# OHDSI/bayes-bridge

Measured on AMD Instinct MI355X. Metric: Gibbs iters/sec (cg sampler), higher is better.
Workload: dtype f64

## Files before the change

bayes-bridge_amd/csrc/cg_sampler.hip:

```cpp
#include <sys/prctl.h>
#include <time.h>

#include "common.hpp"
#include "philox.hpp"
#include "tiled_layout.hpp"

namespace bbx {

int launch_cg_setup(bbx_design* h, int n_unshrunk, const double* phi,
                    const double* sd, const double* x0, double* s, double* d,
                    double* xs, CGState* st, double atol);
int launch_cg_direction(bbx_design* h, int k, CGState* st,
                        const double* rr_part, const double* r, double* pvec,
                        const double* s, double* sp, double* c_part,
                        const double* d = nullptr, double* pdp_part = nullptr,
                        unsigned long long* word = nullptr,
                        unsigned long long tag = 0);
int launch_cg_update(bbx_design* h, int k, CGState* st, const double* pq_part,
                     const double* pvec, const double* q, double* x, double* r,
                     double* rr_part);
int launch_cg_finish(bbx_design* h, const double* s, const double* x,
                     double* coef);

__global__ __launch_bounds__(256) void fill_normal_kernel(
// ... 15 lines not shown
    nz = nz || (x[i] != 0.);
  if (nz) atomicOr(flag, 1);
}

int launch_fill_normal(bbx_design* h, int64_t len, uint64_t seed,
                       uint64_t stream, double* d_out, bool prio,
                       hipStream_t on) {
  int64_t nb = (len + 255) / 256;
  if (nb > 4096) nb = 4096;
  if (nb < 1) nb = 1;
  BBX_LAUNCH(fill_normal_kernel, dim3((unsigned)nb), dim3(256), 0,
                     on ? on : h->stream, len, seed, stream, d_out,
                     prio ? 1 : 0);
  BBX_HIP(hipGetLastError());
  return BBX_OK;
}

struct CGUpdate {
  int k;
  CGState* st;
  double* x;
  double* r;
  bool* merged;
};
static int apply_operator(bbx_design* h, const double* d_omega,
                          const double* sp, const double* x, const double* s,
                          const double* d, double* q,
                          const CGUpdate* upd = nullptr) {
  TdotEpilogue ep;
  ep.mode = TD_OPER;
// ... 58 lines not shown
  double* sp = h->w_P[6].as<double>() + (h->intercept ? 1 : 0);
  CGState* st = h->cg_state.as<CGState>();
  const bool fold = tiled_fold_applies(h);
  double* sr = h->w_P[9].as<double>() + (h->intercept ? 1 : 0);
  double* tu = h->w_n[2].as<double>();

  if (d_eta1 == nullptr) {
    double* e1 = h->w_n[2].as<double>();
    double* e2 = h->w_P[8].as<double>();
    BBX_TRY(launch_fill_normal(h, h->n, seed, STREAM_ETA1, e1));
    BBX_TRY(launch_fill_normal(h, h->P, seed, STREAM_ETA2, e2));
    d_eta1 = e1;
    d_eta2 = e2;
  }

  BBX_TRY(launch_cg_setup(h, n_unshrunk, d_phi, d_sd, d_x0, s, d, x, st, atol));

  CGState* host_st = static_cast<CGState*>(h->host_pinned);
  if (x0_zero < 0) {
    int* d_flag = &st->pad;
    int* h_flag = reinterpret_cast<int*>(host_st);
    BBX_HIP(hipMemsetAsync(d_flag, 0, sizeof(int), h->stream));
    BBX_LAUNCH(any_nonzero_kernel, dim3(NPART), dim3(256), 0,
                       h->stream, h->P, d_x0, d_flag);
    BBX_HIP(hipGetLastError());
    BBX_HIP(hipMemcpyAsync(h_flag, d_flag, sizeof(int), hipMemcpyDeviceToHost,
                           h->stream));
    BBX_HIP(hipStreamSynchronize(h->stream));
    x0_zero = (*h_flag == 0) ? 1 : 0;
  }

// ... 1 lines not shown
    double* w = h->w_n[1].as<double>();
    TdotEpilogue ep;
    ep.mode = TD_RESID;
    ep.s = s;
    ep.d = d;
    ep.x = x0_zero ? nullptr : x;
    ep.z = d_z;
    ep.phi = d_phi;
    ep.eta2 = d_eta2;
    ep.dot_part = part_slot(h, PS_RR);
    if (fold) {
      ep.fold_sr = sr;
      ep.fold_cr_part = part_slot(h, PS_C);
    }
    if (!x0_zero && !h->sparse && dense_fused_applies(h)) {
      BBX_TRY(launch_prep_v(h, x, s, sp, part_slot(h, PS_C)));
      BBX_TRY(launch_sqrt_scale(h, d_omega, d_eta1, w, part_slot(h, PS_SUMW),
                                nullptr, true));
      const int st_f =
          launch_operator_dense_fused(h, sp, d_omega, ep, r, nullptr, w);
      if (st_f != 0)
        return st_f < 0 ? st_f
                        : fail(BBX_ERR_STATE,
                               "single-pass dense operator refused its design");
    } else {
      const double* t0 = nullptr;
      if (!x0_zero) {
        double* t = h->w_n[0].as<double>();
        BBX_TRY(launch_prep_v(h, x, s, sp, part_slot(h, PS_C)));
        BBX_TRY(launch_dot(h, sp, d_omega, t, nullptr));
        t0 = t;
      }
      BBX_TRY(launch_sqrt_scale(h, d_omega, d_eta1, w, part_slot(h, PS_SUMW),
                                t0, t0 == nullptr));
      BBX_TRY(launch_tdot(h, w, part_slot(h, PS_SUMW), ep, r));
    }
  }


  struct SkipScope {
    bbx_design* h;
    ~SkipScope() { h->skip_flag = nullptr; }
  } skip_scope{h};
  h->skip_flag = &st->done;
  double* pdp = part_slot(h, PS_PDP);
  bool merged = false;
  h->cg_serial += 1;
  const unsigned long long tag = (h->cg_serial & 0xFFFFFFull) << CG_WORD_TAG_SHIFT;
  unsigned long long* const word = h->cg_word_dev;
  volatile unsigned long long* const hword = h->cg_word_host;
  struct TagScope {
    bbx_design* h;
// ... 185 lines not shown
```

bayes-bridge_amd/csrc/chain.hip:

```cpp
#include <cmath>
#include <new>
#include <vector>

#include "chain.hpp"
#include "philox.hpp"
#include "samplers.hpp"
#include "pg_queue.hpp"

namespace bbx {

__device__ inline double wsum(double x) { return wave_allsum(x); }

__device__ inline double block_total_256(double x) {
  __shared__ double s_w[256 / WAVE];
  x = wsum(x);
  if ((threadIdx.x & (WAVE - 1)) == 0) s_w[threadIdx.x / WAVE] = x;
  __syncthreads();
  double r = 0.;
  if (threadIdx.x == 0)
    for (int k = 0; k < 256 / WAVE; ++k) r += s_w[k];
  __syncthreads();
  return r;
}

// ... 27 lines not shown
      prior_sd = shrunk_scale(g, lscale[j - nu], slab);
      guess *= prior_sd;
    }
    phi[j] = 1. / prior_sd;
    x0[j] = guess;
    double est = 1.;
    if (n_avg > 1) {
      const double k = (double)n_avg;
      const double m = mean[j];
      const double var = k / (k - 1.) * (square[j] - m * m);
      const double w = (k - 1.) / (k - 1. + 5.);
      est = sqrt(w * var + (1. - w) * 1.);
    }
    sd[j] = est;
    z[j] = zs * zbase[j];
  }
}

#define BBX_BRANCH_PRIO() do { if (prio) __builtin_amdgcn_s_setprio(3); } while (0)
static int lscale_prio() {
  static const int on = getenv("BBX_LSCALE_PRIO") ? atoi(getenv("BBX_LSCALE_PRIO")) : 1;
  return on;
}
static int branch_prio() {
  static const int on = !(getenv("BBX_BRANCH_PRIO") && atoi(getenv("BBX_BRANCH_PRIO")) == 0);
  return on;
}
__global__ __launch_bounds__(256) void chain_summary_kernel(
    int64_t P, int nu, double slab, long long n_avg,
    const ChainScalars* __restrict__ sc, const double* __restrict__ lscale,
// ... 129 lines not shown
    } else {
      const double xf = x / sd_unshrunk[j];
      c += xf * xf;
    }
  }
  const double ta = block_total_256(a);
  const double tb = block_total_256(b);
  const double tc = block_total_256(c);
  if (threadIdx.x == 0) {
    part_pow[blockIdx.x] = ta;
    part_slab[blockIdx.x] = tb;
    part_fixed[blockIdx.x] = tc;
  }
}

__global__ __launch_bounds__(256) void chain_gscale_kernel(
    int64_t n_shrunk, int nu, double alpha, double shape0, double rate0,
    double lower_bd, int update_mode, uint64_t seed, uint64_t stream,
    const double* __restrict__ part_pow, const double* __restrict__ part_slab,
    const double* __restrict__ part_fixed,
    const double* __restrict__ sd_unshrunk, ChainScalars* __restrict__ sc,
    int prio) {
  BBX_BRANCH_PRIO();
  const double pow_sum = sum_row_parts(part_pow, NPART);
  const double slab_sum = sum_row_parts(part_slab, NPART);
  const double fixed_sum = sum_row_parts(part_fixed, NPART);
  if (threadIdx.x != 0) return;
  double g = sc->gscale;
  if (n_shrunk > 0) {
    if (update_mode == BBX_GSCALE_OPTIMIZE) {
      const double ph = (double)n_shrunk / alpha / pow_sum;
      g = pow(ph, -(1. / alpha));
    } else if (update_mode == BBX_GSCALE_SAMPLE) {
      if (pow_sum == 0.) {
        g = 0.;
      } else {
        const double shape = shape0 + (double)n_shrunk / alpha;
        const double rate = rate0 + pow_sum;
        Philox rng(seed, stream, 0);
        const double ph = gamma_draw(rng, shape) / rate;
        g = 1. / pow(ph, 1. / alpha);
      }
    }
    if (update_mode != BBX_GSCALE_FIXED && g < lower_bd) {
      g = lower_bd;
      sc->n_gscale_clamped += 1;
    }
  } else {
    g = 1.;
  }
  sc->gscale = g;
  sc->abs_pow_sum = pow_sum;
  double lp = -.5 * slab_sum;
  double prior = 0.;
  if (n_shrunk > 0)
    prior += -(double)n_shrunk * log(g) - pow_sum / pow(g, alpha);
  prior += -.5 * fixed_sum;
  for (int j = 0; j < nu; ++j)
    if (sd_unshrunk[j] < INFINITY) prior -= log(sd_unshrunk[j]);
  prior += (shape0 - 1.) * log(g) - rate0 * g;
  sc->logprior = lp + prior;
}

constexpr int TS_BLOCK = 256;
constexpr int TS_MAX_COPIES = 16;
constexpr unsigned TS_MAX_TRIAL = 4095u;

template <class Store>
__device__ inline void tilted_stable_block(int64_t base, int64_t count,
                                           double a, uint64_t seed,
                                           uint64_t stream,
                                           const double* s_tilt,
                                           double cost_threshold, Store store) {
  __shared__ int s_pending[TS_BLOCK];
  __shared__ int s_next_dr[TS_BLOCK];
  __shared__ int s_next_dc[TS_BLOCK];
// ... 57 lines not shown
    if (active && ok && s_winner[item] == c) store(item, val);
    if (tid < m) {
      const int it = s_pending[tid];
      if (s_winner[it] == 0x7fffffff) {
        s_tried[it] += (unsigned)copies;
        if (tid < n_dr)
          s_next_dr[atomicAdd(&s_n_dr, 1)] = it;
        else
          s_next_dc[atomicAdd(&s_n_dc, 1)] = it;
      }
    }
    __syncthreads();
  }
}

__global__ __launch_bounds__(TS_BLOCK) void chain_lscale_kernel(
    int64_t n_shrunk, int nu, double alpha, uint64_t seed, uint64_t stream,
    ChainScalars* __restrict__ sc, const double* __restrict__ coef,
    double* __restrict__ lscale, int items, double cost_threshold, int prio) {
  __shared__ double s_tilt[TS_BLOCK];
  BBX_BRANCH_PRIO();
  const double g = sc->gscale;
  for (int64_t base = (int64_t)blockIdx.x * items; base < n_shrunk;
       base += (int64_t)gridDim.x * items) {
    const int64_t count =
        (n_shrunk - base < items) ? (n_shrunk - base) : items;
    if (alpha == 2.) {
      if (threadIdx.x < count) lscale[base + threadIdx.x] = .5;
      continue;
    }
    if (threadIdx.x < count) {
      const double r = coef[base + threadIdx.x + nu] / g;
      s_tilt[threadIdx.x] = r * r;
    }
    __syncthreads();
    tilted_stable_block(base, count, alpha / 2., seed, stream, s_tilt,
                        cost_threshold, [&](int item, double ts) {
// ... 68 lines not shown
static double ts_cost_threshold() { return TiltedStable::kCostThreshold; }

static inline uint64_t iter_stream(uint64_t stream, int64_t iter) {
  return stream | ((uint64_t)iter << 8);
}

static int grid_for(int64_t len, int cap) {
  int64_t nb = (len + 255) / 256;
  if (nb > cap) nb = cap;
  if (nb < 1) nb = 1;
  return (int)nb;
}

static int chain_linear_predictor(bbx_chain* c) {
  bbx_design* h = c->h;
  BBX_TRY(launch_prep_v(h, c->coef.as<double>(), nullptr, nullptr,
                        part_slot(h, PS_C), h->skip_flag));
  return launch_dot(h, c->coef.as<double>(), nullptr, c->psi.as<double>(),
                    nullptr);
}

static int chain_tail_hook(void* ctx) {
  return chain_linear_predictor(static_cast<bbx_chain*>(ctx));
}

static bool chain_tail_applies(const bbx_chain* c) {
  static const bool on = !(getenv("BBX_CHAIN_TAIL") && atoi(getenv("BBX_CHAIN_TAIL")) == 0);
  const bbx_design* h = c->h;
  if (!on || !h->sparse || h->format != BBX_FORMAT_TILED || h->hybrid) return false;
  int G = 0;
  return tiled_describe(h, 0, nullptr, nullptr, nullptr, &G, nullptr, nullptr) ==
             BBX_OK && G == 1;
// ... 17 lines not shown
                     c->n_unshrunk, c->model, c->slab,
                     (long long)c->n_averaged, sc, c->lscale.as<double>(),
                     c->sd_unshrunk.as<double>(), c->mean.as<double>(),
                     c->square.as<double>(), c->zbase.as<double>(),
                     c->phi.as<double>(), c->x0.as<double>(),
                     c->sd.as<double>(), c->z.as<double>(), c->pending_store,
                     c->samp_gscale.as<double>(), c->samp_logp.as<double>());
  c->pending_store = -1;
  if (c->model == BBX_MODEL_LINEAR)
    BBX_LAUNCH(chain_fill_obs_prec_kernel, dim3(grid_for(n, ROW_GRID)),
                       dim3(256), 0, s, n, sc, c->obs_prec.as<double>());
  BBX_HIP(hipGetLastError());
  return BBX_OK;
}

int chain_post_draw(bbx_chain* c, bool have_psi, int phases,
                    bbx_chain* branch_of) {
  bbx_design* h = c->h;
  hipStream_t s = h->stream;
  const int64_t P = h->P, n = h->n;
  const int nu = c->n_unshrunk;
  const int64_t n_shrunk = P - nu;
  ChainScalars* sc = c->scalars.as<ChainScalars>();

  static const int fork_env =
      getenv("BBX_CHAIN_FORK") ? atoi(getenv("BBX_CHAIN_FORK")) : -1;
  const bool fork = fork_env >= 0 ? fork_env == 1
                                  : (n >= 50000 && n_shrunk >= 2048);
  bbx_chain* owner = branch_of ? branch_of : c;
  if (fork && owner->stream2 == nullptr) {
    BBX_HIP(hipStreamCreateWithFlags(&owner->stream2, hipStreamNonBlocking));
  }
  if (fork && c->ev_join == nullptr)
    BBX_HIP(hipEventCreateWithFlags(&c->ev_join, hipEventDisableTiming));
  hipStream_t s_b = !fork ? s : owner->stream2;
  if (h->coef_in_flight) {
    if (fork && (phases & POST_BRANCH))
      BBX_HIP(hipStreamWaitEvent(s_b, h->ev_poll, 0));
    h->coef_in_flight = false;
  }

  if (!have_psi && (phases & POST_BRANCH)) BBX_TRY(chain_linear_predictor(c));

  if (phases & POST_BRANCH) {
  if (c->coef_sampler == BBX_SAMPLER_CG) {
    BBX_LAUNCH(chain_summary_kernel, dim3(NPART), dim3(256), 0, s_b, P,
                       nu, c->slab, (long long)c->n_averaged, sc,
                       c->lscale.as<double>(), c->coef.as<double>(),
                       c->mean.as<double>(), c->square.as<double>(),
                       fork ? branch_prio() : 0);
    c->n_averaged += 1;
  }
  double* pp = c->misc_part.as<double>();
  BBX_LAUNCH(chain_coef_sums_kernel, dim3(NPART), dim3(256), 0, s_b, P,
                     nu, c->bridge_exp, c->slab, c->coef.as<double>(),
                     c->sd_unshrunk.as<double>(), pp, pp + NPART,
                     pp + 2 * NPART, fork ? branch_prio() : 0);
  const double lower_bd = .001 / power_exp_ave_magnitude(c->bridge_exp);
  BBX_LAUNCH(chain_gscale_kernel, dim3(1), dim3(256), 0, s_b, n_shrunk,
                     nu, c->bridge_exp, c->shape0, c->rate0, lower_bd,
                     c->gscale_update, c->seed,
                     iter_stream(STREAM_GSCALE, c->iter), pp, pp + NPART,
                     pp + 2 * NPART, c->sd_unshrunk.as<double>(), sc,
                     fork ? branch_prio() : 0);
  if (n_shrunk > 0) {
    static const int items_env =
        getenv("BBX_TS_ITEMS") ? atoi(getenv("BBX_TS_ITEMS")) : 0;
    const int items = (items_env >= 8 && items_env <= TS_BLOCK) ? items_env
                      : (n_shrunk / TS_BLOCK < 1024) ? 128 : TS_BLOCK;
    int64_t nb = (n_shrunk + items - 1) / items;
    if (nb > 8192) nb = 8192;
    BBX_LAUNCH(chain_lscale_kernel, dim3((unsigned)nb), dim3(TS_BLOCK),
                       0, s_b, n_shrunk, nu, c->bridge_exp, c->seed,
                       iter_stream(STREAM_LSCALE, c->iter), sc,
                       c->coef.as<double>(), c->lscale.as<double>(), items,
                       ts_cost_threshold(), fork ? lscale_prio() : 0);
  }
  }

  hipError_t launch_err = hipSuccess;
  if (phases & POST_MAIN) {
  static const int eta_env =
      getenv("BBX_ETA_AHEAD") ? atoi(getenv("BBX_ETA_AHEAD")) : -1;
  const bool eta_ahead = eta_env >= 0 ? eta_env == 1 : n >= 250000;
  if (eta_ahead && fork && branch_of == nullptr && (phases & POST_JOIN)) {
    if (!c->eta1_next.ptr) {
      BBX_TRY(c->eta1_next.alloc(sizeof(double) * (size_t)n));
      BBX_TRY(c->eta2_next.alloc(sizeof(double) * (size_t)P));
    }
    const uint64_t next_seed = cg_draw_seed(c, (uint64_t)c->iter + 1);
    static const bool fill_prio = !(getenv("BBX_FILL_PRIO") &&
                                    atoi(getenv("BBX_FILL_PRIO")) == 0);
    BBX_TRY(launch_fill_normal(h, n, next_seed, STREAM_ETA1,
                               c->eta1_next.as<double>(), fill_prio));
    BBX_TRY(launch_fill_normal(h, P, next_seed, STREAM_ETA2,
                               c->eta2_next.as<double>(), fill_prio));
    c->eta_iter = c->iter + 1;
  }
  int rg = grid_for(n, ROW_GRID);
  double* rp = c->row_part.as<double>();
  if (c->model == BBX_MODEL_LOGIT) {
    static const int pg_env =
        getenv("BBX_PG_ELEMS") ? atoi(getenv("BBX_PG_ELEMS")) : -1;
    const int elems = pg_env >= 0 ? pg_env : polya_gamma_elems(n);
#define BBX_PG_LAUNCH(KERNEL, PER_BLOCK)                                       \
  do {                                                                         \
    rg = grid_for((n + (PER_BLOCK) - 1) / (PER_BLOCK) * 256, ROW_GRID);        \
    BBX_LAUNCH(KERNEL, dim3(rg), dim3(256), 0, s, n, c->seed,          \
                       iter_stream(STREAM_PG, c->iter),                        \
                       c->outcome.as<double>(), c->n_trial.as<double>(),       \
                       c->psi.as<double>(), c->obs_prec.as<double>(), rp);     \
  } while (0)
    if (elems == 0) BBX_PG_LAUNCH(chain_pg_lane_kernel, 256);
// ... 13 lines not shown

  launch_err = hipGetLastError();
  if (phases & POST_JOIN) {
    if (fork) {
      BBX_HIP(hipEventRecord(c->ev_join, s_b));
      BBX_HIP(hipStreamWaitEvent(s, c->ev_join, 0));
    }
    c->iter += 1;
  }
  BBX_HIP(launch_err);
  return BBX_OK;
}

static int chain_step(bbx_chain* c, int maxiter, double atol, int* n_cg_iter) {
  const uint64_t it = (uint64_t)c->iter;
  BBX_TRY(chain_pre_draw(c));
  int info = 0;
  const bool have_eta = c->eta_iter == (long long)it && c->eta1_next.ptr;
  if (c->coef_sampler == BBX_SAMPLER_CHOLESKY) {
    bbx_design* h = c->h;
    if (!have_eta) {
      if (!c->eta2_next.ptr)
        BBX_TRY(c->eta2_next.alloc(sizeof(double) * (size_t)h->P));
      BBX_TRY(launch_fill_normal(h, h->P, cg_draw_seed(c, it), STREAM_ETA2,
                                 c->eta2_next.as<double>()));
    }
    const bool linear = c->model == BBX_MODEL_LINEAR;
    const int st = chol_sample_device(
        h, linear ? nullptr : c->obs_prec.as<double>(), 1.,
        linear ? &c->scalars.as<ChainScalars>()->obs_prec : nullptr,
        c->phi.as<double>(), c->z.as<double>(), c->eta2_next.as<double>(),
        c->coef.as<double>());
    c->eta_iter = -1;
    if (st < 0) return st;
    c->coef_sample = nullptr;
    if (n_cg_iter) *n_cg_iter = 0;
    BBX_TRY(chain_post_draw(c, false, POST_ALL));
    return 0;
  }
  if (c->coef_sampler == BBX_SAMPLER_WOODBURY) {
    bbx_design* h = c->h;
    if (!have_eta) {
      if (!c->eta1_next.ptr)
        BBX_TRY(c->eta1_next.alloc(sizeof(double) * (size_t)h->n));
      if (!c->eta2_next.ptr)
        BBX_TRY(c->eta2_next.alloc(sizeof(double) * (size_t)h->P));
      BBX_TRY(launch_fill_normal(h, h->n, cg_draw_seed(c, it), STREAM_ETA1,
                                 c->eta1_next.as<double>()));
      BBX_TRY(launch_fill_normal(h, h->P, cg_draw_seed(c, it), STREAM_ETA2,
                                 c->eta2_next.as<double>()));
    }
    const bool linear = c->model == BBX_MODEL_LINEAR;
    const int st = woodbury_sample_device(
        h, linear ? nullptr : c->obs_prec.as<double>(), 1.,
        linear ? &c->scalars.as<ChainScalars>()->obs_prec : nullptr,
        c->phi.as<double>(),
        linear ? c->outcome.as<double>() : c->kappa.as<double>(),
        linear ? 0 : 1, c->eta1_next.as<double>(), c->eta2_next.as<double>(),
        c->coef.as<double>());
    c->eta_iter = -1;
    if (st < 0) return st;
    c->coef_sample = nullptr;
    if (n_cg_iter) *n_cg_iter = 0;
    BBX_TRY(chain_post_draw(c, false, POST_ALL));
    return 0;
  }
  struct TailScope {
    bbx_design* h;
    ~TailScope() {
      h->tail_hook = nullptr;
      h->tail_ctx = nullptr;
      h->coef_copy = nullptr;
    }
  } tail_scope{c->h};
  c->h->coef_copy = c->coef_sample;
  if (chain_tail_applies(c)) {
    c->h->tail_hook = chain_tail_hook;
    c->h->tail_ctx = c;
  }

  int st = cg_sample_device(
      c->h, c->obs_prec.as<double>(), c->phi.as<double>(), c->z.as<double>(),
      c->x0.as<double>(), c->sd.as<double>(), c->n_unshrunk,
      have_eta ? c->eta1_next.as<double>() : nullptr,
      have_eta ? c->eta2_next.as<double>() : nullptr,
      cg_draw_seed(c, it), maxiter, atol, c->coef.as<double>(), n_cg_iter,
      &info, c->mean_zero ? 1 : 0);
  c->eta_iter = -1;
  if (st < 0) return st;
  c->mean_zero = false;
  BBX_TRY(chain_post_draw(c, c->h->tail_ran, POST_ALL));
  c->h->tail_ran = false;
  return info;
}

int chain_begin_run(bbx_chain* c, int n_sample) {
  c->pending_store = -1;
  c->coef_sample = nullptr;
  BBX_TRY(c->samp_gscale.alloc(sizeof(double) * (size_t)(n_sample + 1)));
  BBX_TRY(c->samp_logp.alloc(sizeof(double) * (size_t)(n_sample + 1)));
  return BBX_OK;
}

int chain_save_sample(bbx_chain* c, int idx, double* d_coef, double* d_lscale,
                      double* d_obs_prec) {
  bbx_design* h = c->h;
  const int64_t P = h->P, n = h->n;
// ... 153 lines not shown
  *out = c;
  return BBX_OK;
}

int bbx_chain_destroy(bbx_chain* c) {
  if (!c) return BBX_OK;
  if (c->h && design_alive(c->h)) {
    (void)hipSetDevice(c->h->device);
    (void)hipStreamSynchronize(c->h->stream);
  }
  if (c->stream2) {
    (void)hipStreamSynchronize(c->stream2);
    (void)hipStreamDestroy(c->stream2);
  }
  if (c->ev_join) (void)hipEventDestroy(c->ev_join);
  if (c->pinned) (void)hipHostFree(c->pinned);
  delete c;
  return BBX_OK;
}

static int bbx_chain_set_state_impl(bbx_chain* c, const double* coef,
                        const double* obs_prec, const double* lscale,
                        const double* gscale) {
  BBX_TRY(chain_check(c));
  bbx_design* h = c->h;
  BBX_HIP(hipSetDevice(h->device));
  if (coef)
    BBX_HIP(hipMemcpy(c->coef.ptr, coef, sizeof(double) * (size_t)h->P,
                      hipMemcpyHostToDevice));
  ChainScalars sc;
// ... 457 lines not shown
```

bayes-bridge_amd/csrc/chain.hpp:

```cpp
#pragma once
#include <cmath>

#include "common.hpp"

namespace bbx {

constexpr int ROW_GRID = 2048;

struct alignas(128) ChainScalars {
  double gscale;
  double logprior;
  double abs_pow_sum;
  long long n_gscale_clamped;
  long long n_lscale_fixed;
  alignas(128) double obs_prec;
  double loglik;
  __host__ __device__ double logp() const { return loglik + logprior; }
};

}

struct bbx_chain {
  bbx_design* h = nullptr;
  int model = BBX_MODEL_LOGIT;
// ... 4 lines not shown
  int64_t n_averaged = 0;
  bool mean_zero = true;
  int gscale_update = BBX_GSCALE_SAMPLE;
  int coef_sampler = BBX_SAMPLER_CG;
  void (*progress)(int, void*) = nullptr;
  void* progress_ctx = nullptr;
  int progress_every = 0;
  bbx::DevMem outcome, n_trial, kappa;
  bbx::DevMem zbase;
  bbx::DevMem coef, phi, x0, sd, z, mean, square, sd_unshrunk;
  bbx::DevMem lscale;
  bbx::DevMem obs_prec, psi;
  bbx::DevMem scalars;
  bbx::DevMem row_part;
  bbx::DevMem misc_part;
  bbx::DevMem eta1_next, eta2_next;
  long long eta_iter = -1;
  bbx::DevMem samp_gscale, samp_logp;
  int pending_store = -1;
  double* coef_sample = nullptr;
  void* pinned = nullptr;
  hipStream_t stream2 = nullptr;
  hipEvent_t ev_join = nullptr;
};

namespace bbx {

inline uint64_t cg_draw_seed(const bbx_chain* c, uint64_t it) {
  return c->seed + 0x9E3779B97F4A7C15ull * (it + 1);
}

int chain_pre_draw(bbx_chain* c);
// ... 10 lines not shown
```

bayes-bridge_amd/csrc/common.hpp:

```cpp
#pragma once

#include <hip/hip_runtime.h>
#include <stdint.h>

#include <exception>
#include <new>
#include <string>
#include <vector>

#include "../../include/bbx.h"

#include <atomic>
namespace bbx {
extern std::atomic<unsigned long long> g_launch_count;
}
#define BBX_LAUNCH(...)                                                   \
  do {                                                                    \
    bbx::g_launch_count.fetch_add(1, std::memory_order_relaxed);          \
    hipLaunchKernelGGL(__VA_ARGS__);                                      \
  } while (0)
#define BBX_LAUNCH_EXT(...)                                               \
  do {                                                                    \
    bbx::g_launch_count.fetch_add(1, std::memory_order_relaxed);          \
    hipExtLaunchKernelGGL(__VA_ARGS__);                                   \
// ... 174 lines not shown
  bbx::DevMem cg_state;
  bbx::DevMem stage_n, stage_P;
  void* host_pinned = nullptr;

  int64_t n_dot = 0, n_tdot = 0;
  int last_cg_iter = 0;
  unsigned long long* cg_word_host = nullptr;
  unsigned long long* cg_word_dev = nullptr;
  unsigned long long cg_serial = 0;
  int cg_recent[8] = {0, 0, 0, 0, 0, 0, 0, 0};
  int cg_recent_n = 0;
  int64_t cg_period_ns = 0;
  bool coef_in_flight = false;
  int64_t cg_empty_launches = 0, cg_solves = 0, cg_naps = 0;
  double* coef_copy = nullptr;
  int (*tail_hook)(void*) = nullptr;
  void* tail_ctx = nullptr;
  bool tail_ran = false;
  hipEvent_t ev_poll = nullptr;
  bool in_operator = false;
  uint64_t operator_serial = 0;
  int cg_fold = -1;
  const int* skip_flag = nullptr;
  bbx::KernelTimer timer;
};

namespace bbx {

enum PartSlot {
  PS_C = 0,
// ... 187 lines not shown
                           const double* d_pps, const double* d_y, int y_is_wy,
                           const double* d_delta, const double* d_xi,
                           double* d_coef_out);
double* wb_stage(bbx_design* h, int k);
void woodbury_release(bbx_design* h);
int launch_dot_dense(bbx_design* h, const double* d_v, const double* d_rowscale,
                     double* d_t);
int launch_tdot_dense(bbx_design* h, const double* d_w, const double* d_sumw_part,
                      const TdotEpilogue& ep, double* d_out);
int cg_sample_device(bbx_design* h, const double* d_omega, const double* d_phi,
                     const double* d_z, const double* d_x0,
                     const double* d_sd, int n_unshrunk, const double* d_eta1,
                     const double* d_eta2, uint64_t seed, int maxiter,
                     double atol, double* d_coef, int* n_iter_out,
                     int* info_out, int x0_zero = -1);

}
```

bayes-bridge_amd/csrc/vecops.hip:

```cpp
#include "common.hpp"

namespace bbx {

std::atomic<unsigned long long> g_launch_count{0};


__device__ inline double wave_sum_v(double x) { return wave_allsum(x); }

__device__ inline void block_store_partial(double x, double* part) {
  __shared__ double s_w[VEC_BLOCK / WAVE];
  x = wave_sum_v(x);
  if ((threadIdx.x & (WAVE - 1)) == 0) s_w[threadIdx.x / WAVE] = x;
  __syncthreads();
  if (threadIdx.x == 0) {
    double r = 0.;
#pragma unroll
    for (int k = 0; k < VEC_BLOCK / WAVE; ++k) r += s_w[k];
    part[blockIdx.x] = r;
  }
  __syncthreads();
}

__device__ inline double sum_partials_v(const double* part) {
  __shared__ double s_tot;
// ... 99 lines not shown
                      const double* d_minus, bool negate) {
  BBX_LAUNCH(sqrt_scale_kernel, dim3(NPART), dim3(VEC_BLOCK), 0,
                     h->stream, h->n, d_omega, d_eta, d_w, d_part, d_minus,
                     negate ? 1 : 0);
  BBX_HIP(hipGetLastError());
  return BBX_OK;
}


__global__ __launch_bounds__(VEC_BLOCK) void cg_setup_kernel(
    int64_t P, int n_unshrunk, const double* __restrict__ phi,
    const double* __restrict__ sd, const double* __restrict__ x0,
    double* __restrict__ s, double* __restrict__ d, double* __restrict__ xs,
    CGState* __restrict__ st, double atol) {
  if (blockIdx.x == 0 && threadIdx.x == 0) {
    st->rho[0] = st->rho[1] = 0.;
    st->atol = atol;
    st->bnorm2 = 0.;
    st->n_iter = 0;
    st->done = 0;
    st->bad = 0;
    st->pad = 0;
    st->running = 1;
    st->pad2 = 0;
  }
  for (int64_t jj = (int64_t)blockIdx.x * VEC_BLOCK + threadIdx.x; jj < P;
       jj += (int64_t)gridDim.x * VEC_BLOCK) {
    const double ph = phi[jj];
    const double sj = (jj < n_unshrunk) ? 2. * sd[jj] : 1. / ph;
    const double sp = sj * ph;
    s[jj] = sj;
    d[jj] = sp * sp;
    xs[jj] = x0[jj] / sj;
  }
}

__global__ __launch_bounds__(VEC_BLOCK) void cg_direction_kernel(
    int64_t P, int intercept, int k, CGState* __restrict__ st,
    const double* __restrict__ rr_part, const double* __restrict__ r,
// ... 85 lines not shown
    const double rj = r0 - alpha * q0;
    r[j0] = rj;
    acc += rj * rj;
  }
  for (int64_t jj = j0 + stride; jj < P; jj += stride) {
    x[jj] += alpha * pvec[jj];
    const double rj = r[jj] - alpha * q[jj];
    r[jj] = rj;
    acc += rj * rj;
  }
  block_store_partial(acc, rr_part);
  if (blockIdx.x == 0 && threadIdx.x == 0) st->n_iter = k + 1;
}

__global__ __launch_bounds__(VEC_BLOCK) void cg_finish_kernel(
    int64_t P, const double* __restrict__ s, const double* __restrict__ x,
    double* __restrict__ coef, double* __restrict__ copy) {
  for (int64_t jj = (int64_t)blockIdx.x * VEC_BLOCK + threadIdx.x; jj < P;
       jj += (int64_t)gridDim.x * VEC_BLOCK) {
    const double v = s[jj] * x[jj];
    coef[jj] = v;
    if (copy) copy[jj] = v;
  }
}

int launch_cg_setup(bbx_design* h, int n_unshrunk, const double* phi,
                    const double* sd, const double* x0, double* s, double* d,
                    double* xs, CGState* st, double atol) {
  BBX_LAUNCH(cg_setup_kernel, dim3(NPART), dim3(VEC_BLOCK), 0,
                     h->stream, h->P, n_unshrunk, phi, sd, x0, s, d, xs, st,
                     atol);
  BBX_HIP(hipGetLastError());
  return BBX_OK;
}

int launch_cg_direction(bbx_design* h, int k, CGState* st,
                        const double* rr_part, const double* r, double* pvec,
                        const double* s, double* sp, double* c_part,
// ... 6 lines not shown
  return BBX_OK;
}

int launch_cg_update(bbx_design* h, int k, CGState* st, const double* pq_part,
                     const double* pvec, const double* q, double* x, double* r,
                     double* rr_part) {
  BBX_LAUNCH(cg_update_kernel, dim3(NPART), dim3(VEC_BLOCK), 0,
                     h->stream, h->P, k, st, pq_part, pvec, q, x, r, rr_part);
  BBX_HIP(hipGetLastError());
  return BBX_OK;
}

int launch_cg_finish(bbx_design* h, const double* s, const double* x,
                     double* coef) {
  BBX_LAUNCH(cg_finish_kernel, dim3(NPART), dim3(VEC_BLOCK), 0,
                     h->stream, h->P, s, x, coef, h->coef_copy);
  BBX_HIP(hipGetLastError());
  return BBX_OK;
}

}
```

Baseline: 331.1.

## Fuse chain setup with CG setup, fold gscale into lscale, prefetch next eta

Merges the per-iteration chain pre-draw and CG setup/prep kernels into one chain_setup_kernel. The finish kernel now also computes the offset partial dot, so the linear predictor can skip a prep pass. Coefficient summary and sums become one kernel, and the global-scale draw moves inside the local-scale kernel to drop a single-block launch. For large designs, the next iteration's normal draws are generated early on a side stream with double-buffered eta arrays. The aim is fewer launches and serial gaps per Gibbs step, at the cost of more coupling between stages and every block redundantly recomputing the gscale draw.

```diff
diff --git a/bayes-bridge_amd/csrc/cg_sampler.hip b/bayes-bridge_amd/csrc/cg_sampler.hip
--- a/bayes-bridge_amd/csrc/cg_sampler.hip
+++ b/bayes-bridge_amd/csrc/cg_sampler.hip
@@ -53,6 +53,17 @@
                      prio ? 1 : 0);
   BBX_HIP(hipGetLastError());
   return BBX_OK;
+}
+
+CGSetupTargets cg_setup_targets(const bbx_design* h) {
+  CGSetupTargets t;
+  t.s = h->w_P[0].as<double>();
+  t.d = h->w_P[1].as<double>();
+  t.xs = h->w_P[2].as<double>();
+  t.sp = h->w_P[6].as<double>() + (h->intercept ? 1 : 0);
+  t.c_part = part_slot(h, PS_C);
+  t.st = h->cg_state.as<CGState>();
+  return t;
 }
 
 struct CGUpdate {
@@ -141,7 +152,12 @@
     d_eta2 = e2;
   }
 
-  BBX_TRY(launch_cg_setup(h, n_unshrunk, d_phi, d_sd, d_x0, s, d, x, st, atol));
+  h->coef_c_ready = false;
+  const bool setup_done = h->setup_done;
+  if (setup_done && x0_zero < 0)
+    return fail(BBX_ERR_INVALID, "a caller's own set-up needs x0_zero given");
+  if (!setup_done)
+    BBX_TRY(launch_cg_setup(h, n_unshrunk, d_phi, d_sd, d_x0, s, d, x, st, atol));
 
   CGState* host_st = static_cast<CGState*>(h->host_pinned);
   if (x0_zero < 0) {
@@ -173,7 +189,7 @@
       ep.fold_cr_part = part_slot(h, PS_C);
     }
     if (!x0_zero && !h->sparse && dense_fused_applies(h)) {
-      BBX_TRY(launch_prep_v(h, x, s, sp, part_slot(h, PS_C)));
+      if (!setup_done) BBX_TRY(launch_prep_v(h, x, s, sp, part_slot(h, PS_C)));
       BBX_TRY(launch_sqrt_scale(h, d_omega, d_eta1, w, part_slot(h, PS_SUMW),
                                 nullptr, true));
       const int st_f =
@@ -186,7 +202,7 @@
       const double* t0 = nullptr;
       if (!x0_zero) {
         double* t = h->w_n[0].as<double>();
-        BBX_TRY(launch_prep_v(h, x, s, sp, part_slot(h, PS_C)));
+        if (!setup_done) BBX_TRY(launch_prep_v(h, x, s, sp, part_slot(h, PS_C)));
         BBX_TRY(launch_dot(h, sp, d_omega, t, nullptr));
         t0 = t;
       }
@@ -195,6 +211,7 @@
       BBX_TRY(launch_tdot(h, w, part_slot(h, PS_SUMW), ep, r));
     }
   }
+  if (h->resid_hook) BBX_TRY(h->resid_hook(h->resid_ctx));
 
 
   struct SkipScope {
diff --git a/bayes-bridge_amd/csrc/chain.hip b/bayes-bridge_amd/csrc/chain.hip
--- a/bayes-bridge_amd/csrc/chain.hip
+++ b/bayes-bridge_amd/csrc/chain.hip
@@ -65,6 +65,67 @@
     }
     sd[j] = est;
     z[j] = zs * zbase[j];
+  }
+}
+
+__global__ __launch_bounds__(256) void chain_setup_kernel(
+    int64_t P, int nu, int model, double slab, long long n_avg,
+    const ChainScalars* __restrict__ sc, const double* __restrict__ lscale,
+    const double* __restrict__ sd_unshrunk, const double* __restrict__ mean,
+    const double* __restrict__ square, const double* __restrict__ zbase,
+    double* __restrict__ phi, double* __restrict__ x0, double* __restrict__ sd,
+    double* __restrict__ z, int store_idx, double* __restrict__ samp_gs,
+    double* __restrict__ samp_lp, int intercept,
+    const double* __restrict__ offset, int warm, double* __restrict__ s,
+    double* __restrict__ d, double* __restrict__ xs, double* __restrict__ sp,
+    double* __restrict__ c_part, CGState* __restrict__ st, double atol) {
+  const double g = sc->gscale;
+  const double zs = (model == BBX_MODEL_LINEAR) ? sc->obs_prec : 1.;
+  if (blockIdx.x == 0 && threadIdx.x == 0) {
+    if (store_idx >= 0) {
+      samp_gs[store_idx] = g;
+      samp_lp[store_idx] = sc->logp();
+    }
+    cg_state_reset(st, atol);
+  }
+  double acc = 0.;
+  for (int64_t j = (int64_t)blockIdx.x * 256 + threadIdx.x; j < P;
+       j += (int64_t)gridDim.x * 256) {
+    double prior_sd, guess = mean[j];
+    if (j < nu) {
+      prior_sd = sd_unshrunk[j];
+    } else {
+      prior_sd = shrunk_scale(g, lscale[j - nu], slab);
+      guess *= prior_sd;
+    }
+    const double ph = 1. / prior_sd;
+    phi[j] = ph;
+    x0[j] = guess;
+    double est = 1.;
+    if (n_avg > 1) {
+      const double k = (double)n_avg;
+      const double m = mean[j];
+      const double var = k / (k - 1.) * (square[j] - m * m);
+      const double w = (k - 1.) / (k - 1. + 5.);
+      est = sqrt(w * var + (1. - w) * 1.);
+    }
+    sd[j] = est;
+    z[j] = zs * zbase[j];
+    const double sj = (j < nu) ? 2. * est : 1. / ph;
+    const double sph = sj * ph;
+    s[j] = sj;
+    d[j] = sph * sph;
+    const double xj = guess / sj;
+    xs[j] = xj;
+    if (warm) {
+      const double val = xj * sj;
+      sp[j] = val;
+      if (j >= intercept) acc += offset[j - intercept] * val;
+    }
+  }
+  if (warm) {
+    const double tot = block_total_256(acc);
+    if (threadIdx.x == 0) c_part[blockIdx.x] = tot;
   }
 }
 
@@ -224,19 +285,51 @@
   }
 }
 
-__global__ __launch_bounds__(256) void chain_gscale_kernel(
-    int64_t n_shrunk, int nu, double alpha, double shape0, double rate0,
-    double lower_bd, int update_mode, uint64_t seed, uint64_t stream,
-    const double* __restrict__ part_pow, const double* __restrict__ part_slab,
-    const double* __restrict__ part_fixed,
-    const double* __restrict__ sd_unshrunk, ChainScalars* __restrict__ sc,
-    int prio) {
+__global__ __launch_bounds__(256) void chain_summary_sums_kernel(
+    int64_t P, int nu, double alpha, double slab, long long n_avg,
+    int summarise, const ChainScalars* __restrict__ sc,
+    const double* __restrict__ lscale, const double* __restrict__ coef,
+    const double* __restrict__ sd_unshrunk, double* __restrict__ mean,
+    double* __restrict__ square, double* __restrict__ part_pow,
+    double* __restrict__ part_slab, double* __restrict__ part_fixed, int prio) {
   BBX_BRANCH_PRIO();
-  const double pow_sum = sum_row_parts(part_pow, NPART);
-  const double slab_sum = sum_row_parts(part_slab, NPART);
-  const double fixed_sum = sum_row_parts(part_fixed, NPART);
-  if (threadIdx.x != 0) return;
-  double g = sc->gscale;
+  const double g = sc->gscale;
+  const double w = 1. / (1. + (double)n_avg);
+  double a = 0., b = 0., c = 0.;
+  for (int64_t j = (int64_t)blockIdx.x * 256 + threadIdx.x; j < P;
+       j += (int64_t)gridDim.x * 256) {
+    const double x = coef[j];
+    if (summarise) {
+      double theta = x;
+      if (j >= nu) theta /= shrunk_scale(g, lscale[j - nu], slab);
+      mean[j] = w * theta + (1. - w) * mean[j];
+      square[j] = w * theta * theta + (1. - w) * square[j];
+    }
+    const double xs = x / slab;
+    b += xs * xs;
+    if (j >= nu) {
+      a += pow(fabs(x), alpha);
+    } else {
+      const double xf = x / sd_unshrunk[j];
+      c += xf * xf;
+    }
+  }
+  const double ta = block_total_256(a);
+  const double tb = block_total_256(b);
+  const double tc = block_total_256(c);
+  if (threadIdx.x == 0) {
+    part_pow[blockIdx.x] = ta;
+    part_slab[blockIdx.x] = tb;
+    part_fixed[blockIdx.x] = tc;
+  }
+}
+
+__device__ inline double gscale_draw(double g, int64_t n_shrunk, double alpha,
+                                     double shape0, double rate0,
+                                     double lower_bd, int update_mode,
+                                     uint64_t seed, uint64_t stream,
+                                     double pow_sum, bool* clamped) {
+  *clamped = false;
   if (n_shrunk > 0) {
     if (update_mode == BBX_GSCALE_OPTIMIZE) {
       const double ph = (double)n_shrunk / alpha / pow_sum;
@@ -254,11 +347,21 @@
     }
     if (update_mode != BBX_GSCALE_FIXED && g < lower_bd) {
       g = lower_bd;
-      sc->n_gscale_clamped += 1;
+      *clamped = true;
     }
   } else {
     g = 1.;
   }
+  return g;
+}
+
+__device__ inline void gscale_store(ChainScalars* __restrict__ sc, double g,
+                                    bool clamped, int64_t n_shrunk, int nu,
+                                    double alpha, double shape0, double rate0,
+                                    double pow_sum, double slab_sum,
+                                    double fixed_sum,
+                                    const double* __restrict__ sd_unshrunk) {
+  if (clamped) sc->n_gscale_clamped += 1;
   sc->gscale = g;
   sc->abs_pow_sum = pow_sum;
   double lp = -.5 * slab_sum;
@@ -270,6 +373,26 @@
     if (sd_unshrunk[j] < INFINITY) prior -= log(sd_unshrunk[j]);
   prior += (shape0 - 1.) * log(g) - rate0 * g;
   sc->logprior = lp + prior;
+}
+
+__global__ __launch_bounds__(256) void chain_gscale_kernel(
+    int64_t n_shrunk, int nu, double alpha, double shape0, double rate0,
+    double lower_bd, int update_mode, uint64_t seed, uint64_t stream,
+    const double* __restrict__ part_pow, const double* __restrict__ part_slab,
+    const double* __restrict__ part_fixed,
+    const double* __restrict__ sd_unshrunk, ChainScalars* __restrict__ sc,
+    int prio) {
+  BBX_BRANCH_PRIO();
+  const double pow_sum = sum_row_parts(part_pow, NPART);
+  const double slab_sum = sum_row_parts(part_slab, NPART);
+  const double fixed_sum = sum_row_parts(part_fixed, NPART);
+  if (threadIdx.x != 0) return;
+  bool clamped;
+  const double g = gscale_draw(sc->gscale, n_shrunk, alpha, shape0, rate0,
+                               lower_bd, update_mode, seed, stream, pow_sum,
+                               &clamped);
+  gscale_store(sc, g, clamped, n_shrunk, nu, alpha, shape0, rate0, pow_sum,
+               slab_sum, fixed_sum, sd_unshrunk);
 }
 
 constexpr int TS_BLOCK = 256;
@@ -357,13 +480,47 @@
   }
 }
 
+struct GscaleInKernel {
+  const double* part_pow = nullptr;
+  const double* part_slab = nullptr;
+  const double* part_fixed = nullptr;
+  const double* sd_unshrunk = nullptr;
+  double shape0 = 0., rate0 = 0., lower_bd = 0.;
+  int update_mode = 0;
+  uint64_t stream = 0;
+};
+
 __global__ __launch_bounds__(TS_BLOCK) void chain_lscale_kernel(
     int64_t n_shrunk, int nu, double alpha, uint64_t seed, uint64_t stream,
     ChainScalars* __restrict__ sc, const double* __restrict__ coef,
-    double* __restrict__ lscale, int items, double cost_threshold, int prio) {
+    double* __restrict__ lscale, int items, double cost_threshold, int prio,
+    GscaleInKernel tau) {
   __shared__ double s_tilt[TS_BLOCK];
+  __shared__ double s_gscale;
   BBX_BRANCH_PRIO();
-  const double g = sc->gscale;
+  double g;
+  if (tau.part_pow) {
+    const double pow_sum = sum_row_parts(tau.part_pow, NPART);
+    double slab_sum = 0., fixed_sum = 0.;
+    if (blockIdx.x == 0) {
+      slab_sum = sum_row_parts(tau.part_slab, NPART);
+      fixed_sum = sum_row_parts(tau.part_fixed, NPART);
+    }
+    if (threadIdx.x == 0) {
+      bool clamped;
+      const double gn = gscale_draw(sc->gscale, n_shrunk, alpha, tau.shape0,
+                                    tau.rate0, tau.lower_bd, tau.update_mode,
+                                    seed, tau.stream, pow_sum, &clamped);
+      s_gscale = gn;
+      if (blockIdx.x == 0)
+        gscale_store(sc, gn, clamped, n_shrunk, nu, alpha, tau.shape0,
+                     tau.rate0, pow_sum, slab_sum, fixed_sum, tau.sd_unshrunk);
+    }
+    __syncthreads();
+    g = s_gscale;
+  } else {
+    g = sc->gscale;
+  }
   for (int64_t base = (int64_t)blockIdx.x * items; base < n_shrunk;
        base += (int64_t)gridDim.x * items) {
     const int64_t count =
@@ -462,8 +619,10 @@
 
 static int chain_linear_predictor(bbx_chain* c) {
   bbx_design* h = c->h;
-  BBX_TRY(launch_prep_v(h, c->coef.as<double>(), nullptr, nullptr,
-                        part_slot(h, PS_C), h->skip_flag));
+  if (!h->coef_c_ready)
+    BBX_TRY(launch_prep_v(h, c->coef.as<double>(), nullptr, nullptr,
+                          part_slot(h, PS_C), h->skip_flag));
+  h->coef_c_ready = false;
   return launch_dot(h, c->coef.as<double>(), nullptr, c->psi.as<double>(),
                     nullptr);
 }
@@ -511,6 +670,66 @@
   return BBX_OK;
 }
 
+static int chain_setup_draw(bbx_chain* c, double atol) {
+  bbx_design* h = c->h;
+  const CGSetupTargets t = cg_setup_targets(h);
+  BBX_LAUNCH(chain_setup_kernel, dim3(NPART), dim3(256), 0, h->stream, h->P,
+                     c->n_unshrunk, c->model, c->slab,
+                     (long long)c->n_averaged,
+                     c->scalars.as<ChainScalars>(), c->lscale.as<double>(),
+                     c->sd_unshrunk.as<double>(), c->mean.as<double>(),
+                     c->square.as<double>(), c->zbase.as<double>(),
+                     c->phi.as<double>(), c->x0.as<double>(),
+                     c->sd.as<double>(), c->z.as<double>(), c->pending_store,
+                     c->samp_gscale.as<double>(), c->samp_logp.as<double>(),
+                     h->intercept, h->offset.as<double>(),
+                     c->mean_zero ? 0 : 1, t.s, t.d, t.xs, t.sp, t.c_part,
+                     t.st, atol);
+  c->pending_store = -1;
+  if (c->model == BBX_MODEL_LINEAR)
+    BBX_LAUNCH(chain_fill_obs_prec_kernel, dim3(grid_for(h->n, ROW_GRID)),
+                       dim3(256), 0, h->stream, h->n,
+                       c->scalars.as<ChainScalars>(), c->obs_prec.as<double>());
+  BBX_HIP(hipGetLastError());
+  return BBX_OK;
+}
+
+static bool chain_forks(const bbx_chain* c) {
+  static const int fork_env =
+      getenv("BBX_CHAIN_FORK") ? atoi(getenv("BBX_CHAIN_FORK")) : -1;
+  return fork_env >= 0 ? fork_env == 1
+                       : (c->h->n >= 50000 && c->h->P - c->n_unshrunk >= 2048);
+}
+
+static bool chain_eta_ahead(const bbx_chain* c) {
+  static const int eta_env =
+      getenv("BBX_ETA_AHEAD") ? atoi(getenv("BBX_ETA_AHEAD")) : -1;
+  return chain_forks(c) && (eta_env >= 0 ? eta_env == 1 : c->h->n >= 250000);
+}
+
+static int chain_resid_hook(void* ctx) {
+  bbx_chain* c = static_cast<bbx_chain*>(ctx);
+  bbx_design* h = c->h;
+  const int64_t next = c->iter + 1;
+  const int b = (int)(next & 1);
+  if (c->stream2 == nullptr)
+    BBX_HIP(hipStreamCreateWithFlags(&c->stream2, hipStreamNonBlocking));
+  if (c->ev_eta == nullptr)
+    BBX_HIP(hipEventCreateWithFlags(&c->ev_eta, hipEventDisableTiming));
+  if (!c->eta1_next[b].ptr)
+    BBX_TRY(c->eta1_next[b].alloc(sizeof(double) * (size_t)h->n));
+  if (!c->eta2_next[b].ptr)
+    BBX_TRY(c->eta2_next[b].alloc(sizeof(double) * (size_t)h->P));
+  const uint64_t next_seed = cg_draw_seed(c, (uint64_t)next);
+  BBX_TRY(launch_fill_normal(h, h->n, next_seed, STREAM_ETA1,
+                             c->eta1_next[b].as<double>(), false, c->stream2));
+  BBX_TRY(launch_fill_normal(h, h->P, next_seed, STREAM_ETA2,
+                             c->eta2_next[b].as<double>(), false, c->stream2));
+  BBX_HIP(hipEventRecord(c->ev_eta, c->stream2));
+  c->eta_iter = next;
+  return BBX_OK;
+}
+
 int chain_post_draw(bbx_chain* c, bool have_psi, int phases,
                     bbx_chain* branch_of) {
   bbx_design* h = c->h;
@@ -520,10 +739,7 @@
   const int64_t n_shrunk = P - nu;
   ChainScalars* sc = c->scalars.as<ChainScalars>();
 
-  static const int fork_env =
-      getenv("BBX_CHAIN_FORK") ? atoi(getenv("BBX_CHAIN_FORK")) : -1;
-  const bool fork = fork_env >= 0 ? fork_env == 1
-                                  : (n >= 50000 && n_shrunk >= 2048);
+  const bool fork = chain_forks(c);
   bbx_chain* owner = branch_of ? branch_of : c;
   if (fork && owner->stream2 == nullptr) {
     BBX_HIP(hipStreamCreateWithFlags(&owner->stream2, hipStreamNonBlocking));
@@ -540,26 +756,39 @@
   if (!have_psi && (phases & POST_BRANCH)) BBX_TRY(chain_linear_predictor(c));
 
   if (phases & POST_BRANCH) {
-  if (c->coef_sampler == BBX_SAMPLER_CG) {
-    BBX_LAUNCH(chain_summary_kernel, dim3(NPART), dim3(256), 0, s_b, P,
-                       nu, c->slab, (long long)c->n_averaged, sc,
-                       c->lscale.as<double>(), c->coef.as<double>(),
-                       c->mean.as<double>(), c->square.as<double>(),
+  double* pp = c->misc_part.as<double>();
+  const bool summarise = c->coef_sampler == BBX_SAMPLER_CG;
+  const double lower_bd = .001 / power_exp_ave_magnitude(c->bridge_exp);
+  const bool short_head =
+      branch_of == nullptr && n_shrunk > 0 && c->bridge_exp != 2.;
+  if (short_head) {
+    BBX_LAUNCH(chain_summary_sums_kernel, dim3(NPART), dim3(256), 0, s_b, P,
+                       nu, c->bridge_exp, c->slab, (long long)c->n_averaged,
+                       summarise ? 1 : 0, sc, c->lscale.as<double>(),
+                       c->coef.as<double>(), c->sd_unshrunk.as<double>(),
+                       c->mean.as<double>(), c->square.as<double>(), pp,
+                       pp + NPART, pp + 2 * NPART, fork ? branch_prio() : 0);
+    if (summarise) c->n_averaged += 1;
+  } else {
+    if (summarise) {
+      BBX_LAUNCH(chain_summary_kernel, dim3(NPART), dim3(256), 0, s_b, P,
+                         nu, c->slab, (long long)c->n_averaged, sc,
+                         c->lscale.as<double>(), c->coef.as<double>(),
+                         c->mean.as<double>(), c->square.as<double>(),
+                         fork ? branch_prio() : 0);
+      c->n_averaged += 1;
+    }
+    BBX_LAUNCH(chain_coef_sums_kernel, dim3(NPART), dim3(256), 0, s_b, P,
+                       nu, c->bridge_exp, c->slab, c->coef.as<double>(),
+                       c->sd_unshrunk.as<double>(), pp, pp + NPART,
+                       pp + 2 * NPART, fork ? branch_prio() : 0);
+    BBX_LAUNCH(chain_gscale_kernel, dim3(1), dim3(256), 0, s_b, n_shrunk,
+                       nu, c->bridge_exp, c->shape0, c->rate0, lower_bd,
+                       c->gscale_update, c->seed,
+                       iter_stream(STREAM_GSCALE, c->iter), pp, pp + NPART,
+                       pp + 2 * NPART, c->sd_unshrunk.as<double>(), sc,
                        fork ? branch_prio() : 0);
-    c->n_averaged += 1;
-  }
-  double* pp = c->misc_part.as<double>();
-  BBX_LAUNCH(chain_coef_sums_kernel, dim3(NPART), dim3(256), 0, s_b, P,
-                     nu, c->bridge_exp, c->slab, c->coef.as<double>(),
-                     c->sd_unshrunk.as<double>(), pp, pp + NPART,
-                     pp + 2 * NPART, fork ? branch_prio() : 0);
-  const double lower_bd = .001 / power_exp_ave_magnitude(c->bridge_exp);
-  BBX_LAUNCH(chain_gscale_kernel, dim3(1), dim3(256), 0, s_b, n_shrunk,
-                     nu, c->bridge_exp, c->shape0, c->rate0, lower_bd,
-                     c->gscale_update, c->seed,
-                     iter_stream(STREAM_GSCALE, c->iter), pp, pp + NPART,
-                     pp + 2 * NPART, c->sd_unshrunk.as<double>(), sc,
-                     fork ? branch_prio() : 0);
+  }
   if (n_shrunk > 0) {
     static const int items_env =
         getenv("BBX_TS_ITEMS") ? atoi(getenv("BBX_TS_ITEMS")) : 0;
@@ -567,33 +796,28 @@
                       : (n_shrunk / TS_BLOCK < 1024) ? 128 : TS_BLOCK;
     int64_t nb = (n_shrunk + items - 1) / items;
     if (nb > 8192) nb = 8192;
+    GscaleInKernel tau;
+    if (short_head) {
+      tau.part_pow = pp;
+      tau.part_slab = pp + NPART;
+      tau.part_fixed = pp + 2 * NPART;
+      tau.sd_unshrunk = c->sd_unshrunk.as<double>();
+      tau.shape0 = c->shape0;
+      tau.rate0 = c->rate0;
+      tau.lower_bd = lower_bd;
+      tau.update_mode = c->gscale_update;
+      tau.stream = iter_stream(STREAM_GSCALE, c->iter);
+    }
     BBX_LAUNCH(chain_lscale_kernel, dim3((unsigned)nb), dim3(TS_BLOCK),
                        0, s_b, n_shrunk, nu, c->bridge_exp, c->seed,
                        iter_stream(STREAM_LSCALE, c->iter), sc,
                        c->coef.as<double>(), c->lscale.as<double>(), items,
-                       ts_cost_threshold(), fork ? lscale_prio() : 0);
+                       ts_cost_threshold(), fork ? lscale_prio() : 0, tau);
   }
   }
 
   hipError_t launch_err = hipSuccess;
   if (phases & POST_MAIN) {
-  static const int eta_env =
-      getenv("BBX_ETA_AHEAD") ? atoi(getenv("BBX_ETA_AHEAD")) : -1;
-  const bool eta_ahead = eta_env >= 0 ? eta_env == 1 : n >= 250000;
-  if (eta_ahead && fork && branch_of == nullptr && (phases & POST_JOIN)) {
-    if (!c->eta1_next.ptr) {
-      BBX_TRY(c->eta1_next.alloc(sizeof(double) * (size_t)n));
-      BBX_TRY(c->eta2_next.alloc(sizeof(double) * (size_t)P));
-    }
-    const uint64_t next_seed = cg_draw_seed(c, (uint64_t)c->iter + 1);
-    static const bool fill_prio = !(getenv("BBX_FILL_PRIO") &&
-                                    atoi(getenv("BBX_FILL_PRIO")) == 0);
-    BBX_TRY(launch_fill_normal(h, n, next_seed, STREAM_ETA1,
-                               c->eta1_next.as<double>(), fill_prio));
-    BBX_TRY(launch_fill_normal(h, P, next_seed, STREAM_ETA2,
-                               c->eta2_next.as<double>(), fill_prio));
-    c->eta_iter = c->iter + 1;
-  }
   int rg = grid_for(n, ROW_GRID);
   double* rp = c->row_part.as<double>();
   if (c->model == BBX_MODEL_LOGIT) {
@@ -637,24 +861,31 @@
 
 static int chain_step(bbx_chain* c, int maxiter, double atol, int* n_cg_iter) {
   const uint64_t it = (uint64_t)c->iter;
-  BBX_TRY(chain_pre_draw(c));
+  bbx_design* h = c->h;
+  const bool cg = c->coef_sampler == BBX_SAMPLER_CG;
+  if (cg)
+    BBX_TRY(chain_setup_draw(c, atol));
+  else
+    BBX_TRY(chain_pre_draw(c));
   int info = 0;
-  const bool have_eta = c->eta_iter == (long long)it && c->eta1_next.ptr;
+  bbx::DevMem& eta1 = c->eta1_next[it & 1];
+  bbx::DevMem& eta2 = c->eta2_next[it & 1];
+  const bool have_eta =
+      c->eta_iter == (long long)it && eta1.ptr && eta2.ptr && c->ev_eta;
+  c->eta_iter = -1;
+  if (have_eta) BBX_HIP(hipStreamWaitEvent(h->stream, c->ev_eta, 0));
   if (c->coef_sampler == BBX_SAMPLER_CHOLESKY) {
-    bbx_design* h = c->h;
     if (!have_eta) {
-      if (!c->eta2_next.ptr)
-        BBX_TRY(c->eta2_next.alloc(sizeof(double) * (size_t)h->P));
+      if (!eta2.ptr) BBX_TRY(eta2.alloc(sizeof(double) * (size_t)h->P));
       BBX_TRY(launch_fill_normal(h, h->P, cg_draw_seed(c, it), STREAM_ETA2,
-                                 c->eta2_next.as<double>()));
+                                 eta2.as<double>()));
     }
     const bool linear = c->model == BBX_MODEL_LINEAR;
     const int st = chol_sample_device(
         h, linear ? nullptr : c->obs_prec.as<double>(), 1.,
         linear ? &c->scalars.as<ChainScalars>()->obs_prec : nullptr,
-        c->phi.as<double>(), c->z.as<double>(), c->eta2_next.as<double>(),
+        c->phi.as<double>(), c->z.as<double>(), eta2.as<double>(),
         c->coef.as<double>());
-    c->eta_iter = -1;
     if (st < 0) return st;
     c->coef_sample = nullptr;
     if (n_cg_iter) *n_cg_iter = 0;
@@ -662,16 +893,13 @@
     return 0;
   }
   if (c->coef_sampler == BBX_SAMPLER_WOODBURY) {
-    bbx_design* h = c->h;
     if (!have_eta) {
-      if (!c->eta1_next.ptr)
-        BBX_TRY(c->eta1_next.alloc(sizeof(double) * (size_t)h->n));
-      if (!c->eta2_next.ptr)
-        BBX_TRY(c->eta2_next.alloc(sizeof(double) * (size_t)h->P));
+      if (!eta1.ptr) BBX_TRY(eta1.alloc(sizeof(double) * (size_t)h->n));
+      if (!eta2.ptr) BBX_TRY(eta2.alloc(sizeof(double) * (size_t)h->P));
       BBX_TRY(launch_fill_normal(h, h->n, cg_draw_seed(c, it), STREAM_ETA1,
-                                 c->eta1_next.as<double>()));
+                                 eta1.as<double>()));
       BBX_TRY(launch_fill_normal(h, h->P, cg_draw_seed(c, it), STREAM_ETA2,
-                                 c->eta2_next.as<double>()));
+                                 eta2.as<double>()));
     }
     const bool linear = c->model == BBX_MODEL_LINEAR;
     const int st = woodbury_sample_device(
@@ -679,41 +907,48 @@
         linear ? &c->scalars.as<ChainScalars>()->obs_prec : nullptr,
         c->phi.as<double>(),
         linear ? c->outcome.as<double>() : c->kappa.as<double>(),
-        linear ? 0 : 1, c->eta1_next.as<double>(), c->eta2_next.as<double>(),
+        linear ? 0 : 1, eta1.as<double>(), eta2.as<double>(),
         c->coef.as<double>());
-    c->eta_iter = -1;
     if (st < 0) return st;
     c->coef_sample = nullptr;
     if (n_cg_iter) *n_cg_iter = 0;
     BBX_TRY(chain_post_draw(c, false, POST_ALL));
     return 0;
   }
-  struct TailScope {
+  struct SolveScope {
     bbx_design* h;
-    ~TailScope() {
+    ~SolveScope() {
       h->tail_hook = nullptr;
       h->tail_ctx = nullptr;
+      h->resid_hook = nullptr;
+      h->resid_ctx = nullptr;
       h->coef_copy = nullptr;
-    }
-  } tail_scope{c->h};
-  c->h->coef_copy = c->coef_sample;
+      h->setup_done = false;
+      h->coef_c_ready = false;
+    }
+  } solve_scope{h};
+  h->coef_copy = c->coef_sample;
+  h->setup_done = true;
   if (chain_tail_applies(c)) {
-    c->h->tail_hook = chain_tail_hook;
-    c->h->tail_ctx = c;
+    h->tail_hook = chain_tail_hook;
+    h->tail_ctx = c;
+  }
+  if (chain_eta_ahead(c)) {
+    h->resid_hook = chain_resid_hook;
+    h->resid_ctx = c;
   }
 
   int st = cg_sample_device(
-      c->h, c->obs_prec.as<double>(), c->phi.as<double>(), c->z.as<double>(),
+      h, c->obs_prec.as<double>(), c->phi.as<double>(), c->z.as<double>(),
       c->x0.as<double>(), c->sd.as<double>(), c->n_unshrunk,
-      have_eta ? c->eta1_next.as<double>() : nullptr,
-      have_eta ? c->eta2_next.as<double>() : nullptr,
+      have_eta ? eta1.as<double>() : nullptr,
+      have_eta ? eta2.as<double>() : nullptr,
       cg_draw_seed(c, it), maxiter, atol, c->coef.as<double>(), n_cg_iter,
       &info, c->mean_zero ? 1 : 0);
-  c->eta_iter = -1;
   if (st < 0) return st;
   c->mean_zero = false;
-  BBX_TRY(chain_post_draw(c, c->h->tail_ran, POST_ALL));
-  c->h->tail_ran = false;
+  BBX_TRY(chain_post_draw(c, h->tail_ran, POST_ALL));
+  h->tail_ran = false;
   return info;
 }
 
@@ -897,6 +1132,7 @@
     (void)hipStreamDestroy(c->stream2);
   }
   if (c->ev_join) (void)hipEventDestroy(c->ev_join);
+  if (c->ev_eta) (void)hipEventDestroy(c->ev_eta);
   if (c->pinned) (void)hipHostFree(c->pinned);
   delete c;
   return BBX_OK;
diff --git a/bayes-bridge_amd/csrc/chain.hpp b/bayes-bridge_amd/csrc/chain.hpp
--- a/bayes-bridge_amd/csrc/chain.hpp
+++ b/bayes-bridge_amd/csrc/chain.hpp
@@ -42,8 +42,9 @@
   bbx::DevMem scalars;
   bbx::DevMem row_part;
   bbx::DevMem misc_part;
-  bbx::DevMem eta1_next, eta2_next;
+  bbx::DevMem eta1_next[2], eta2_next[2];
   long long eta_iter = -1;
+  hipEvent_t ev_eta = nullptr;
   bbx::DevMem samp_gscale, samp_logp;
   int pending_store = -1;
   double* coef_sample = nullptr;
diff --git a/bayes-bridge_amd/csrc/common.hpp b/bayes-bridge_amd/csrc/common.hpp
--- a/bayes-bridge_amd/csrc/common.hpp
+++ b/bayes-bridge_amd/csrc/common.hpp
@@ -212,6 +212,10 @@
   bool coef_in_flight = false;
   int64_t cg_empty_launches = 0, cg_solves = 0, cg_naps = 0;
   double* coef_copy = nullptr;
+  bool coef_c_ready = false;
+  bool setup_done = false;
+  int (*resid_hook)(void*) = nullptr;
+  void* resid_ctx = nullptr;
   int (*tail_hook)(void*) = nullptr;
   void* tail_ctx = nullptr;
   bool tail_ran = false;
@@ -429,5 +433,25 @@
                      const double* d_eta2, uint64_t seed, int maxiter,
                      double atol, double* d_coef, int* n_iter_out,
                      int* info_out, int x0_zero = -1);
-
-}
+struct CGSetupTargets {
+  double* s;
+  double* d;
+  double* xs;
+  double* sp;
+  double* c_part;
+  CGState* st;
+};
+CGSetupTargets cg_setup_targets(const bbx_design* h);
+__device__ inline void cg_state_reset(CGState* st, double atol) {
+  st->rho[0] = st->rho[1] = 0.;
+  st->atol = atol;
+  st->bnorm2 = 0.;
+  st->n_iter = 0;
+  st->done = 0;
+  st->bad = 0;
+  st->pad = 0;
+  st->running = 1;
+  st->pad2 = 0;
+}
+
+}
diff --git a/bayes-bridge_amd/csrc/vecops.hip b/bayes-bridge_amd/csrc/vecops.hip
--- a/bayes-bridge_amd/csrc/vecops.hip
+++ b/bayes-bridge_amd/csrc/vecops.hip
@@ -137,15 +137,7 @@
     double* __restrict__ s, double* __restrict__ d, double* __restrict__ xs,
     CGState* __restrict__ st, double atol) {
   if (blockIdx.x == 0 && threadIdx.x == 0) {
-    st->rho[0] = st->rho[1] = 0.;
-    st->atol = atol;
-    st->bnorm2 = 0.;
-    st->n_iter = 0;
-    st->done = 0;
-    st->bad = 0;
-    st->pad = 0;
-    st->running = 1;
-    st->pad2 = 0;
+    cg_state_reset(st, atol);
   }
   for (int64_t jj = (int64_t)blockIdx.x * VEC_BLOCK + threadIdx.x; jj < P;
        jj += (int64_t)gridDim.x * VEC_BLOCK) {
@@ -261,14 +253,19 @@
 }
 
 __global__ __launch_bounds__(VEC_BLOCK) void cg_finish_kernel(
-    int64_t P, const double* __restrict__ s, const double* __restrict__ x,
-    double* __restrict__ coef, double* __restrict__ copy) {
+    int64_t P, int intercept, const double* __restrict__ s,
+    const double* __restrict__ x, const double* __restrict__ offset,
+    double* __restrict__ coef, double* __restrict__ copy,
+    double* __restrict__ c_part) {
+  double acc = 0.;
   for (int64_t jj = (int64_t)blockIdx.x * VEC_BLOCK + threadIdx.x; jj < P;
        jj += (int64_t)gridDim.x * VEC_BLOCK) {
     const double v = s[jj] * x[jj];
     coef[jj] = v;
     if (copy) copy[jj] = v;
-  }
+    if (jj >= intercept) acc += offset[jj - intercept] * v;
+  }
+  block_store_partial(acc, c_part);
 }
 
 int launch_cg_setup(bbx_design* h, int n_unshrunk, const double* phi,
@@ -305,9 +302,12 @@
 int launch_cg_finish(bbx_design* h, const double* s, const double* x,
                      double* coef) {
   BBX_LAUNCH(cg_finish_kernel, dim3(NPART), dim3(VEC_BLOCK), 0,
-                     h->stream, h->P, s, x, coef, h->coef_copy);
-  BBX_HIP(hipGetLastError());
-  return BBX_OK;
-}
-
-}
+                     h->stream, h->P, h->intercept, s, x,
+                     h->offset.as<double>(), coef, h->coef_copy,
+                     part_slot(h, PS_C));
+  BBX_HIP(hipGetLastError());
+  h->coef_c_ready = true;
+  return BBX_OK;
+}
+
+}
```

Result: no change. 330.5 (median of 2 runs) (-0.2%).
